# HKUST-KnowComp/DualMessagePassing

Measured on AMD Instinct MI355X. Metric: (pattern,graph) pairs/sec DMPNN fwd+bwd hid=128, higher is better.
Workload: dtype f32

## Files before the change

dualmessagepassing_amd/_abi.py:

```python
import ctypes

c_int = ctypes.c_int
c_i32 = ctypes.c_int32
c_i64 = ctypes.c_int64
c_u64 = ctypes.c_uint64
c_f32 = ctypes.c_float
c_double = ctypes.c_double
c_ptr = ctypes.c_void_p
c_size = ctypes.c_size_t

ABI_VERSION = 97

DMP_COLLATE_MAX_JOBS = 4
DMP_POOL_MAX_JOBS = 4
DMP_REDUCE_MAX_SEGMENTS = 16
DMP_ADAMW_MAX_SKIP = 16
DMP_ADAMW_MAX_SEGMENTS = 1024
DMP_LOOKUP_MAX_JOBS = 8
DMP_CONCAT_MAX_JOBS = 12
DMP_GEMM_MAX_JOBS = 12
DMP_GEMM_MAX_TERMS = 3
DMP_ATB_MAX_JOBS = 8
DMP_MEM_MEAN, DMP_MEM_SUM, DMP_MEM_MAX = 0, 1, 2
DMP_LRP_MAX_NEIGHBOURS = 32
# ... 282 lines not shown
    "dmp_typed_partial_rows": (c_i64, [c_i64, c_int]),
    "dmp_out_fwd_typed": (c_int, [_p(dmp_typed_job), c_int, c_ptr, c_ptr, c_ptr, c_i64, c_i64, c_int, c_ptr]),
    "dmp_bwd_h1_typed": (c_int, [c_ptr, c_i64, c_ptr, c_i64, c_ptr, c_i64, c_ptr, c_ptr, c_ptr, c_i64, c_i64, c_int, c_f32, c_ptr, c_i64,
                                 c_ptr, c_ptr, c_ptr]),
    "dmp_kept_rows_jobs": (c_int, [_p(dmp_kept_job), c_int, c_ptr, c_ptr, c_ptr, c_ptr, c_i64, c_ptr, c_ptr, c_ptr, c_ptr]),
    "dmp_row_mask_bits_jobs": (c_int, [_p(dmp_rowmask_job), c_int, c_ptr]),
    "dmp_atb2_blocks": (c_i64, [c_i64, c_int]),
    "dmp_atb2_jobs": (c_int, [_p(dmp_atb2_job), c_int, c_ptr, c_ptr, c_ptr, c_i64, c_i64, c_int, c_ptr]),
    "dmp_bwd_z_w": (c_int, [c_ptr, c_i64, c_ptr, c_i64, c_ptr, c_i64, c_ptr, c_i64, c_i64, c_ptr, c_i64, c_ptr, c_ptr, c_f32, c_f32,
                            c_ptr, c_ptr, c_ptr, c_i64, c_i64, c_int, c_ptr, c_i64, c_ptr, c_i64, c_ptr, c_ptr]),
    "dmp_out_fwd_typed_codes": (c_int, [_p(dmp_typed_job), c_ptr, c_i64, c_int, c_ptr, c_i64, c_i64, c_i64, c_ptr, c_ptr, c_ptr, c_i64, c_i64, c_int, c_ptr]),
    "dmp_bwd_h1_w_blocks": (c_i64, [c_i64]),
    "dmp_bwd_h1_w": (c_int, [c_ptr, c_i64, c_ptr, c_i64, c_ptr, c_i64, c_ptr, c_ptr, c_i64, c_i64, c_int, c_f32, c_ptr, c_i64,
                             c_ptr, c_ptr, c_ptr, c_ptr]),
    "dmp_node_chain_blocks": (c_i64, [c_i64]),
    "dmp_node_chain_panel_words": (c_i64, []),
    "dmp_node_chain_pack": (c_int, [_p(dmp_chain_panel), c_int, c_ptr, c_ptr]),
    "dmp_node_chain_fwd": (c_int, [c_ptr, c_i64, c_ptr, c_i64, c_ptr, c_ptr, c_ptr, c_int, c_f32, c_ptr, c_ptr, c_i64, c_i64, c_int,
                                   c_ptr, c_i64, c_ptr, c_i64, c_ptr, c_i64, c_ptr]),
    "dmp_node_chain_bwd": (c_int, [c_ptr, c_i64, c_ptr, c_i64, c_ptr, c_i64, c_ptr, c_int, c_f32, c_ptr, c_ptr, c_i64, c_i64, c_int,
                                   c_ptr, c_i64, c_ptr, c_i64, c_ptr, c_i64, c_ptr, c_ptr, c_ptr]),
    "dmp_edge_mlp_fwd": (c_int, [c_ptr, c_i64, c_ptr, c_i64, c_ptr, c_i64, c_i64, c_ptr, c_ptr, c_ptr, c_ptr, c_i64, c_int, c_ptr, c_ptr, c_i64,
                                 c_ptr, c_ptr, c_ptr, c_i64, c_i64, c_int, c_f32, c_ptr, c_i64, c_ptr, c_i64, c_ptr]),
    "dmp_row_mask_bits": (c_int, [c_ptr, c_i64, c_ptr, c_ptr]),
    "dmp_row_mask_rows": (c_int, [c_ptr, c_i64, c_int, c_i64, c_ptr, c_ptr]),
    "dmp_bwd_z_fused": (c_int, [c_ptr, c_i64, c_ptr, c_i64, c_ptr, c_i64, c_i64, c_ptr, c_i64, c_ptr, c_ptr, c_ptr,
                                c_f32, c_f32, c_i64, c_int, c_ptr, c_i64, c_ptr]),
    "dmp_gemm_k128": (c_int, [c_ptr, c_i64, c_ptr, c_i64, c_int, c_ptr, c_i64, c_i64, c_int, c_ptr]),
    "dmp_edge_combine": (c_int, [c_ptr, c_i64, c_ptr, c_i64, c_ptr, c_ptr, c_ptr, c_ptr, c_ptr, c_i64,
                                 c_int, c_int, c_f32, c_ptr, c_i64, c_ptr]),
    "dmp_relu_bwd_g_colsum": (c_int, [c_ptr, c_i64, c_ptr, c_i64, c_ptr, c_ptr, c_i64, c_int, c_f32, c_ptr, c_i64,
                                      c_ptr, c_ptr]),
    "dmp_edge_combine_bwd_g": (c_int, [c_ptr, c_i64, c_ptr, c_ptr, c_i64, c_int, c_ptr, c_i64, c_ptr]),
    "dmp_compgcn_agg": (c_int, [c_ptr, c_i64, c_ptr, c_i64, c_ptr, c_ptr, c_ptr, c_ptr, c_i64, c_int, c_int,
                                c_ptr, c_i64, c_ptr]),
    "dmp_compgcn_agg_bwd": (c_int, [c_ptr, c_i64, c_ptr, c_i64, c_ptr, c_i64, c_ptr, c_ptr, c_ptr, c_ptr,
                                    c_i64, c_int, c_int, c_ptr, c_i64, c_ptr, c_i64, c_ptr]),
    "dmp_attn_supported_dh": (c_int, [c_int]),
    "dmp_attn_fwd": (c_int, [c_ptr, c_ptr, c_ptr, c_ptr, c_ptr, c_i64, c_i64, c_i64, c_int, c_int, c_f32, c_ptr, c_ptr, c_ptr, c_ptr]),
    "dmp_attn_bwd": (c_int, [c_ptr, c_ptr, c_ptr, c_ptr, c_ptr, c_ptr, c_ptr, c_ptr, c_i64, c_i64, c_i64, c_int, c_int, c_f32, c_ptr,
                             c_ptr, c_ptr, c_ptr, c_ptr]),
    "dmp_mem_init_fwd": (c_int, [c_ptr, c_i64, c_ptr, c_i64, c_ptr, c_i64, c_i64, c_int, c_int, c_int, c_int, c_int, c_ptr, c_ptr,
                                 c_ptr, c_ptr, c_ptr, c_ptr, c_ptr]),
    "dmp_mem_init_bwd": (c_int, [c_ptr, c_ptr, c_ptr, c_ptr, c_ptr, c_i64, c_i64, c_int, c_int, c_int, c_int, c_ptr, c_ptr, c_ptr]),
    "dmp_cnn_fwd": (c_int, [c_ptr, c_i64, c_i64, c_int, c_ptr, c_ptr, c_int, c_int, c_int, c_int, c_int, c_f32, c_ptr, c_int, c_ptr,
                            c_ptr, c_ptr, c_ptr, c_ptr]),
# ... 35 lines not shown
```

dualmessagepassing_amd/_build.py:

```python
import fcntl
import hashlib
import os
import shutil
import subprocess
import tempfile

_HERE = os.path.dirname(os.path.abspath(__file__))
CSRC = os.path.join(_HERE, "csrc")
LIB_PATH = os.path.join(CSRC, "libdmp_hip.so")
HASH_PATH = LIB_PATH + ".srchash"
SOURCES = ["dmp_agg.hip", "dmp_segacc.hip", "dmp_compact.hip", "dmp_graph.hip", "dmp_fused.hip", "dmp_mfma.hip", "dmp_typed.hip", "dmp_h1w.hip", "dmp_nodechain.hip", "dmp_edgemlp.hip", "dmp_atb.hip", "dmp_fold.hip", "dmp_heads.hip", "dmp_layer0.hip", "dmp_bn.hip", "dmp_attn.hip", "dmp_mem.hip", "dmp_cnn.hip", "dmp_rnn.hip", "dmp_relconv.hip", "dmp_relcorr.hip", "dmp_txl.hip", "dmp_match.hip", "dmp_lrp.hip", "dmp_rank.hip", "dmp_rank_typed.hip", "dmp_lrppool.hip",
           "dmp_subiso.cpp"]
HEADERS = ["dmp_common.h", "dmp_mfma_common.h", "dmp_rank_kernel.h", os.path.join("..", "..", "include", "dmp_hip.h")]
ARCH = "gfx950"
FLAGS = ["-O3", "-std=c++17", "-fPIC", "-ffp-contract=off", "-Wall", "-Wno-unused-function"]


def find_hipcc():
    for cand in (os.environ.get("HIPCC"), shutil.which("hipcc"), "/opt/rocm/bin/hipcc"):
        if cand and os.path.exists(cand):
            return cand
    return None


def source_hash():
    h = hashlib.sha256()
    h.update((ARCH + " ".join(FLAGS)).encode())
    for f in SOURCES + HEADERS:
        with open(os.path.join(CSRC, f), "rb") as fh:
            h.update(f.encode())
            h.update(fh.read())
    return h.hexdigest()


# ... 53 lines not shown
```

dualmessagepassing_amd/fused.py:

```python
import ctypes as _ctypes
import os as _os
import threading

import torch
from torch.autograd.function import once_differentiable

from . import _abi, _lib, gatememo, ops
from ._lib import check, ptr, stream_ptr


def _partials(rows, H, dev):
    lib = _lib.load()
    return torch.empty((int(lib.dmp_colsum_partial_rows(rows, H)), H), dtype=torch.float32, device=dev)


MAX_REDUCE_SEGMENTS = _abi.DMP_REDUCE_MAX_SEGMENTS


class _Deferred(threading.local):

    def __init__(self):
        self.stack = []


# ... 544 lines not shown

def l0_rows(l0, W0, z):
    if l0 is None or not getattr(l0, "z_from_codes", False):
        return z
    n, K, H = l0.z_head.size(0), l0.K, W0.size(1)
    out = torch.empty((l0.enc.size(0), H), dtype=torch.float32, device=l0.enc.device)
    out[:n].copy_(l0.z_head)
    if out.size(0) > n:
        smallk_embed(l0.enc[n:, :K], W0.detach()[-K:], None, out[n:], H)
    return out


USE_OUT_CODES = True


def out_codes_ok(h1, enc, K, Wc):
    lib = _lib.load()
    lim = (1 << 32) - 65536
    return bool(USE_OUT_CODES and h1.size(1) == 128 and not lib.dmp_dev_get_exact_fp32() and 1 <= K <= 16 and Wc.size(0) == K and Wc.size(1) == 128
                and enc.dtype == torch.float32 and enc.stride(1) == 1 and enc.stride(0) % 4 == 0 and enc.data_ptr() % 16 == 0
                and enc.size(0) == h1.size(0) and h1.size(0) * 128 * 4 < lim and Wc.stride(1) == 1)


def out_fwd_typed_codes(h1, W2t, b2, enc, K, Wc, tiles, prev=None, out=None, w_in_out=True, row0=0):
    lib = _lib.load()
    slot_edge, tile_scale, num_tiles, bound = tiles
    R, H = h1.shape
    if out is None:
        out = dead_rows_buffer((R, H), h1.device)
    Wc = Wc.detach()
    _lib.require_gpu(h1, W2t, out, prev, b2, enc, Wc)
    j = _abi.dmp_typed_job()
    j.Hin, j.ldh, j.W2, j.ldw, j.w_in_out = h1.data_ptr(), h1.stride(0), W2t.data_ptr(), W2t.stride(0), int(bool(w_in_out))
    j.bias = ptr(b2)
    j.R, j.ldr = ptr(prev), (prev.stride(0) if prev is not None else H)
    j.R2, j.ldr2 = None, H
    j.act, j.slope = 0, 0.0
    j.out, j.ldo = out.data_ptr(), out.stride(0)
    with _lib.timed("out_fwd_typed_codes[H=%d,R=%d]", (H, R), 4 * H * R * 2 + 4 * enc.size(1) * R):
        check(lib.dmp_out_fwd_typed_codes(_ctypes.byref(j), ptr(enc), enc.stride(0), int(K), ptr(Wc), Wc.stride(0), int(row0),
                                          0 if prev is None else min(R, prev.size(0)), ptr(slot_edge), ptr(tile_scale),
                                          ptr(num_tiles), bound, R, H, stream_ptr()), "dmp_out_fwd_typed_codes")
    return out


def out_fwd_typed(h1, W2t, b2, prev, tiles, out=None, w_in_out=True, slope=None, prev2=None, first=None):
    R, H = h1.shape
    if out is None:
        out = dead_rows_buffer((R, H), h1.device)
    if first is not None:
        if prev2 is not None or slope is not None:
            raise _lib.DmpError("out_fwd_typed(first=...): neither a second addend nor an activation on the result")
        edge_mlp_fwd(first["z"], first["Wes"], first["P"], first["ldp"], first["bias"], first["coef"], first["index"], first["slope"],
                     W2t, b2, prev, tiles, sel=first.get("sel"), w_in_out=w_in_out, h1=h1, out=out)
        return out
    typed_jobs([dict(a=h1, W=W2t, bias=b2, prev=prev, prev2=prev2, out=out, w_in_out=w_in_out, slope=slope)], tiles)
    return out


USE_EDGE_MLP_FWD = True


def edge_mlp_fwd_ok(H, *tensors):
    if not USE_EDGE_MLP_FWD or H != 128 or _lib.load().dmp_dev_get_exact_fp32():
        return False
    lim = (1 << 32) - 65536
    for a in tensors:
        if a is None:
            continue
        if (a.dtype != torch.float32 or a.dim() != 2 or a.stride(1) != 1 or a.stride(0) % 4 or a.stride(0) * 4 > 16383
                or a.data_ptr() % 16 or a.size(0) * a.stride(0) * 4 >= lim):
            return False
    return True


def edge_mlp_fwd(z, Wes, P, ldp, bias, coef, index, slope, W2t, b2, prev, tiles, sel=None, w_in_out=True, h1=None, out=None):
    lib = _lib.load()
    E, H = z.shape
    slot_edge, tile_scale, num_tiles, bound = tiles
    if h1 is None:
        h1 = dead_rows_buffer((E, H), z.device)
    if out is None:
        out = dead_rows_buffer((E, H), z.device)
    Wes = Wes.contiguous()
    sel_a, sel_b = (sel[0], sel[1]) if sel is not None else index.edge_select(coef)[:2]
    _lib.require_gpu(z, Wes, P, bias, W2t, b2, prev, h1, out)
    with _lib.timed("edge_fwd_typed[H=%d,E=%d]", (H, E), 4 * H * (2 * E + 2 * index.num_nodes) + 12 * E):
        check(lib.dmp_edge_mlp_fwd(ptr(z), z.stride(0), ptr(Wes), Wes.size(1), ptr(P), ldp, index.num_nodes, ptr(bias), ptr(sel_a), ptr(sel_b),
                                   ptr(W2t), W2t.stride(0), int(bool(w_in_out)), ptr(b2), ptr(prev), prev.stride(0) if prev is not None else H,
                                   ptr(slot_edge), ptr(tile_scale), ptr(num_tiles), bound, E, H, float(slope), ptr(h1), h1.stride(0),
                                   ptr(out), out.stride(0), stream_ptr()), "dmp_edge_mlp_fwd")
    return h1, out


def bwd_h1_typed(d_o, W2, h1, tiles, slope=0.0, out=None):
    lib = _lib.load()
# ... 423 lines not shown
    return gatememo.memo(v_gate, "node_rows", (index,), build)


L0_NODE_MAX_COLS = 40


def l0_node_pack(VK, K0, H, Mv, Ma, Mb):
    W = torch.zeros((L0_NODE_MAX_COLS, 3 * H), dtype=torch.float32, device=Mv.device)
    W[:VK] = Mv
    W[VK:VK + K0, :H] = Ma
    W[VK + K0:VK + 2 * K0, :H] = Mb
    return W


def l0_node_fwd(venc, VK, S0, K0, Kp, W, bias, slope, mask, n0, n1, H, h1, P, rows=None, q_begin=0):
    lib = _lib.load()
    lst, cnt = rows if (rows is not None and mask is not None) else (None, None)
    with _lib.timed("l0_node_fwd[K=%d,R=%d]", (VK + 2 * K0, n1 - n0), 4 * (3 * H + VK + 2 * K0) * (n1 - n0)):
        check(lib.dmp_l0_node_fwd(ptr(venc), venc.stride(0), VK, ptr(S0), S0.stride(0), K0, Kp, ptr(W), W.stride(0), ptr(bias), float(slope),
                                  ptr(mask), ptr(lst), ptr(cnt), 0 if lst is None else lst.numel(), min(int(q_begin), n0), n0, n1, H,
                                  ptr(h1), h1.stride(0), ptr(P), P.stride(0), stream_ptr()), "dmp_l0_node_fwd")


def l0_edge_fwd(enc, K, M, P, ldp, bias, coef, index, slope=0.0, rows=None, out=None, mask=None):
    lib = _lib.load()
    E, H = enc.size(0), M.size(1) // 2
    if out is None:
        out = torch.empty((E, H), dtype=torch.float32, device=enc.device)
    r0, r1 = (0, E) if rows is None else rows
    sel_a, sel_b, coef_e = index.edge_select(coef)
    if mask is not None and r0 % 32 != 0:
        mask = None
    if mask is not None and l0_row_list(r0, r1 - r0):
        lst, cnt = kept_rows(mask, r0, r1)
        with _lib.timed("l0_edge_fwd[K=%d,E=%d]", (K, r1 - r0), 4 * H * (r1 - r0 + min(2 * index.num_nodes, 2 * (r1 - r0))) + (4 * enc.size(1) + 12) * (r1 - r0)):
            check(lib.dmp_l0_edge_fwd_rows(ptr(enc[r0:]), enc.stride(0), K, ptr(M), M.stride(0), ptr(P), ldp, ptr(bias), ptr(coef_e[r0:]),
                                           ptr(sel_a[r0:]), ptr(sel_b[r0:]), ptr(lst), ptr(cnt), r1 - r0, H, slope, ptr(out[r0:]),
                                           out.stride(0), stream_ptr()), "dmp_l0_edge_fwd_rows")
        return out
    with _lib.timed("l0_edge_fwd[K=%d,E=%d]", (K, r1 - r0), 4 * H * (r1 - r0 + min(2 * index.num_nodes, 2 * (r1 - r0))) + (4 * enc.size(1) + 12) * (r1 - r0)):
        check(lib.dmp_l0_edge_fwd_masked(ptr(enc[r0:]), enc.stride(0), K, ptr(M), M.stride(0), ptr(P), ldp, ptr(bias), ptr(coef_e[r0:]),
                                         ptr(sel_a[r0:]), ptr(sel_b[r0:]), None if mask is None else ptr(mask[r0 // 32:]), r1 - r0, H,
                                         slope, ptr(out[r0:]), out.stride(0), stream_ptr()),
              "dmp_l0_edge_fwd")
    return out


def l0_bwd_w(enc, K, coef_e, d_pre, d_zn=None, rows=None, out=None, mask=None):
    lib = _lib.load()
    E, H = d_pre.shape
    r0, r1 = (0, E) if rows is None else rows
    own = False
    if mask is not None and r0 % 32 != 0:
# ... 377 lines not shown
        if chained:
            pass
        elif nd is not None:
            xn = dead_rows_buffer((N, H), z.device) if (inner & 1) else torch.zeros((N, H), dtype=torch.float32, device=z.device)
            if nW2t is not None:
                out_fwd_typed(H1n, nW2t, nb2, x if residual else None, nd.tiles, out=xn)
            else:
                out_fwd_typed(H1n, nW2, nb2, x if residual else None, nd.tiles, out=xn, w_in_out=False)
        elif onepanel_ok(H):
            xn = out_fwd_mfma(H1n, nW2, nb2, v_gate, x if residual else None, nW2t)
        else:
            xn = gate_residual(x if residual else None, torch.addmm(nb2, H1n, nW2.t()), v_gate)
        sums_only = epool is not None and not edge_rows
        zn = None
        side.wait("erows" if l0 is not None else "tiles")
        dead_gate = e_gate if dead_h1_rows(index, H, e_gate) else None
        dead_in = dead_gate is not None and dead_edge_rows(index, H, e_gate)
        mlp_tiles = None
        if (l0 is None and dead_in and not sums_only and residual and eW2t is not None and (inner & 1)
                and edge_mlp_fwd_ok(H, z, PXr, eW2t)):
            mlp_tiles = live_tiles(index, coef, e_gate)
        if l0 is not None:
            H1e = dead_rows_buffer((z.size(0), H), z.device) if dead_gate is not None else torch.empty((z.size(0), H), dtype=torch.float32, device=z.device)
            for t, rows, _ in tables:
                if rows[1] > rows[0]:
                    l0_edge_fwd(enc0, K0, M0[t * K0:(t + 1) * K0], PXr, ldpx, be, coef, index, slope, rows, H1e,
                                mask=gate_row_mask(dead_gate) if dead_gate is not None else None)
        elif mlp_tiles is not None:
            H1e = dead_rows_buffer((z.size(0), H), z.device)
            zn = out_fwd_typed(H1e, eW2t, eb2, z, mlp_tiles,
                               first=dict(z=z, Wes=Wes, P=PXr, ldp=ldpx, bias=be, coef=coef, index=index, slope=slope,
                                          sel=None if nd is None else nd.sel))
        elif typed_ok(index, H):
            H1e = edge_fwd_typed(z, Wes, PXr, ldpx, be, coef, index, slope, dead_gate=dead_gate, sel=None if nd is None else nd.sel)
        elif mfma_ok(index, H):
            H1e = edge_fwd_mfma(z, Wes, PXr, ldpx, be, coef, index, slope)
        else:
            G = z @ Wes
            H1e = edge_combine_raw(G, 2 * H, PXr, ldpx, be, coef, index, H, relu=True, slope=slope)
            del G
            if not sums_only:
                Oe = torch.addmm(eb2, H1e, eW2.t())
                zn = gate_residual(z if residual else None, Oe, e_gate)
        if zn is None and not sums_only:
            dead = (3 if (inner & 1) else 1) if dead_in else 0
            side.wait("tiles")
            lt = live_tiles(index, coef, e_gate) if (dead == 3 and eW2t is not None) else None
            if lt is not None:
                tl_ = ascending_tiles(e_gate) or lt
                if l0 is not None and residual and getattr(l0, "z_from_codes", False) and out_codes_ok(H1e, l0.enc, l0.K, W0[-l0.K:]):
# ... 337 lines not shown
```

include/dmp_hip.h:

```cpp
#ifndef DMP_HIP_H
#define DMP_HIP_H

#include <stddef.h>
#include <stdint.h>

#ifdef __cplusplus
extern "C" {
#endif

#define DMP_OK 0
#define DMP_ERR_BAD_ARG (-1)
#define DMP_ERR_UNSUPPORTED (-2)
#define DMP_ERR_HIP (-3)

#define DMP_ABI_VERSION 97
int dmp_abi_version(void);
const char *dmp_last_hip_error(void);


size_t dmp_csr_workspace_words(int64_t num_nodes, int64_t num_edges);

int dmp_csr_build(const int64_t *key, const uint8_t *flag, int64_t num_edges,
                  int64_t num_nodes, int32_t *rowptr, int32_t *ent,
                  int32_t *key32, int64_t *degree, int32_t *status,
// ... 492 lines not shown
                 const int32_t *slot_edge, const int32_t *num_tiles, int64_t tiles_bound, int64_t E, int H, float slope,
                 float *dG, int64_t ldg, float *partial, float *partial_rows, float *partial_w, void *stream);

typedef struct {
  const float *W; int64_t ld; int transposed;
} dmp_chain_panel;
int64_t dmp_node_chain_blocks(int64_t tiles_bound);
int64_t dmp_node_chain_panel_words(void);
int dmp_node_chain_pack(const dmp_chain_panel *panels, int num_panels, uint32_t *out, void *stream);
int dmp_node_chain_fwd(const float *x, int64_t ldx, const float *S, int64_t lds, const uint32_t *panels, const float *bn, const float *b2,
                       int residual, float slope, const int32_t *slot, const int32_t *num_tiles, int64_t tiles_bound, int64_t rows, int H,
                       float *H1n, int64_t ldh, float *P, int64_t ldp, float *xn, int64_t ldxn, void *stream);
int dmp_node_chain_bwd(const float *dxn, int64_t ldd, const float *H1n, int64_t ldh, const float *dP, int64_t ldp, const uint32_t *panels,
                       int residual, float slope, const int32_t *slot, const int32_t *num_tiles, int64_t tiles_bound, int64_t rows, int H,
                       float *dPn, int64_t ldn, float *dS, int64_t lds, float *dx, int64_t ldx, float *partial, float *partial_rows,
                       void *stream);

int dmp_edge_mlp_fwd(const float *Z, int64_t ldz, const float *W, int64_t ldw, const float *P, int64_t ldp, int64_t num_nodes,
                     const float *bias1, const int32_t *selA, const int32_t *selB, const float *W2, int64_t ldw2, int w2_in_out,
                     const float *bias2, const float *R, int64_t ldr, const int32_t *slot_edge, const float *tile_scale,
                     const int32_t *num_tiles, int64_t tiles_bound, int64_t num_edges, int H, float slope, float *H1, int64_t ldh,
                     float *out, int64_t ldo, void *stream);

int dmp_bwd_z_fused(const float *dPre, int64_t ldp, const float *W, int64_t ldw,
                    const float *D, int64_t ldd, int64_t num_nodes, const float *base, int64_t ldb,
                    const float *coefE, const int32_t *dst, const uint8_t *flag, float s0,
                    float s1, int64_t num_edges, int H, float *dZ, int64_t ldz, void *stream);

int dmp_edge_fwd_typed(const float *Z, int64_t ldz, const float *W, int64_t ldw, const float *P,
                       int64_t ldp, int64_t num_nodes, const float *bias, const int32_t *selA,
                       const int32_t *selB, const int32_t *slot_edge, const float *tile_scale,
                       const int32_t *num_tiles, int64_t tiles_bound, int64_t num_edges, int H,
                       float slope, float *H1, int64_t ldh, void *stream);
int dmp_mask_slots(const int32_t *slot, int64_t n, const float *gate, int64_t E, int32_t *out, void *stream);
int dmp_bwd_z_typed_arow(const float *dPre, int64_t ldp, const float *W, int64_t ldw, const float *D, int64_t ldd,
                         int64_t num_nodes, const float *base, int64_t ldb, const int32_t *dst, const uint8_t *flag,
                         float s0, float s1, const int32_t *slot_edge, const int32_t *slot_arow, const float *tile_scale,
                         const int32_t *num_tiles, int64_t tiles_bound, int64_t E, int H, int w_transposed,
                         const int32_t *base_map, int64_t base_rows, float *dZ, int64_t ldz, void *stream);

int64_t dmp_atb_typed_blocks_h(int64_t tiles_bound, int H);
int dmp_atb_typed(const float *Z, int64_t ldz, const float *dPre, int64_t ldp,
                  const int32_t *slot_edge, const float *tile_scale, const int32_t *num_tiles,
                  int64_t tiles_bound, int64_t num_edges, int H, float *partial_T,
                  float *partial_B, void *stream);

// ... 122 lines not shown
```

Before: 487,900.

## Fuse layer-0 edge MLP first and second GEMMs into one warp-specialized kernel

Adds a new HIP kernel that computes the layer-0 edge first linear layer (from code encodings via small per-table matrices plus gathered node projections), activation, and the second linear layer with code term and residual in a single launch. Producer waves build the hidden tile in LDS while consumer waves run the output GEMM on it, using split-bf16 MFMA emulation of fp32. This is meant to remove the separate l0_edge_fwd and out_fwd_typed_codes launches and the intermediate H1 round trip before the second GEMM. The fused path is gated on operand layout, K limits, tile availability and the residual/codes configuration, so some calls fall back to the old path.

```diff
diff --git a/dualmessagepassing_amd/_abi.py b/dualmessagepassing_amd/_abi.py
--- a/dualmessagepassing_amd/_abi.py
+++ b/dualmessagepassing_amd/_abi.py
@@ -328,6 +328,10 @@
                                    c_ptr, c_i64, c_ptr, c_i64, c_ptr, c_i64, c_ptr, c_ptr, c_ptr]),
     "dmp_edge_mlp_fwd": (c_int, [c_ptr, c_i64, c_ptr, c_i64, c_ptr, c_i64, c_i64, c_ptr, c_ptr, c_ptr, c_ptr, c_i64, c_int, c_ptr, c_ptr, c_i64,
                                  c_ptr, c_ptr, c_ptr, c_i64, c_i64, c_int, c_f32, c_ptr, c_i64, c_ptr, c_i64, c_ptr]),
+    "dmp_l0_edge_mlp_max_codes": (c_int, []),
+    "dmp_l0_edge_mlp_fwd": (c_int, [c_ptr, c_i64, c_int, c_ptr, c_i64, c_int, c_i64, c_ptr, c_i64, c_i64, c_ptr, c_ptr, c_ptr, c_ptr, c_f32,
+                                    c_ptr, c_i64, c_int, c_ptr, c_ptr, c_i64, c_i64, c_ptr, c_i64, c_i64, c_ptr, c_ptr, c_i64, c_i64, c_int,
+                                    c_ptr, c_i64, c_ptr, c_i64, c_ptr]),
     "dmp_row_mask_bits": (c_int, [c_ptr, c_i64, c_ptr, c_ptr]),
     "dmp_row_mask_rows": (c_int, [c_ptr, c_i64, c_int, c_i64, c_ptr, c_ptr]),
     "dmp_bwd_z_fused": (c_int, [c_ptr, c_i64, c_ptr, c_i64, c_ptr, c_i64, c_i64, c_ptr, c_i64, c_ptr, c_ptr, c_ptr,
diff --git a/dualmessagepassing_amd/_build.py b/dualmessagepassing_amd/_build.py
--- a/dualmessagepassing_amd/_build.py
+++ b/dualmessagepassing_amd/_build.py
@@ -9,7 +9,7 @@
 CSRC = os.path.join(_HERE, "csrc")
 LIB_PATH = os.path.join(CSRC, "libdmp_hip.so")
 HASH_PATH = LIB_PATH + ".srchash"
-SOURCES = ["dmp_agg.hip", "dmp_segacc.hip", "dmp_compact.hip", "dmp_graph.hip", "dmp_fused.hip", "dmp_mfma.hip", "dmp_typed.hip", "dmp_h1w.hip", "dmp_nodechain.hip", "dmp_edgemlp.hip", "dmp_atb.hip", "dmp_fold.hip", "dmp_heads.hip", "dmp_layer0.hip", "dmp_bn.hip", "dmp_attn.hip", "dmp_mem.hip", "dmp_cnn.hip", "dmp_rnn.hip", "dmp_relconv.hip", "dmp_relcorr.hip", "dmp_txl.hip", "dmp_match.hip", "dmp_lrp.hip", "dmp_rank.hip", "dmp_rank_typed.hip", "dmp_lrppool.hip",
+SOURCES = ["dmp_agg.hip", "dmp_segacc.hip", "dmp_compact.hip", "dmp_graph.hip", "dmp_fused.hip", "dmp_mfma.hip", "dmp_typed.hip", "dmp_h1w.hip", "dmp_nodechain.hip", "dmp_edgemlp.hip", "dmp_l0mlp.hip", "dmp_atb.hip", "dmp_fold.hip", "dmp_heads.hip", "dmp_layer0.hip", "dmp_bn.hip", "dmp_attn.hip", "dmp_mem.hip", "dmp_cnn.hip", "dmp_rnn.hip", "dmp_relconv.hip", "dmp_relcorr.hip", "dmp_txl.hip", "dmp_match.hip", "dmp_lrp.hip", "dmp_rank.hip", "dmp_rank_typed.hip", "dmp_lrppool.hip",
            "dmp_subiso.cpp"]
 HEADERS = ["dmp_common.h", "dmp_mfma_common.h", "dmp_rank_kernel.h", os.path.join("..", "..", "include", "dmp_hip.h")]
 ARCH = "gfx950"
diff --git a/dualmessagepassing_amd/csrc/dmp_l0mlp.hip b/dualmessagepassing_amd/csrc/dmp_l0mlp.hip
--- /dev/null
+++ b/dualmessagepassing_amd/csrc/dmp_l0mlp.hip
@@ -0,0 +1,378 @@
+#include <type_traits>
+
+#include "dmp_mfma_common.h"
+
+namespace dmp {
+namespace {
+
+struct L0MlpArgs {
+  const float *enc; int64_t lde; int K;
+  const float *M; int64_t ldm; int tables;
+  int64_t row_split;
+  const float *P; int64_t ldp; int64_t num_nodes;
+  const float *bias1;
+  const float *coef_e;
+  const int32_t *selA, *selB;
+  const float *W2; int64_t ldw2; int w2_transposed;
+  const float *bias2;
+  const float *Wc; int64_t ldwc; int64_t code_row0;
+  const float *R; int64_t ldr; int64_t r_rows;
+  float *H1; int64_t ldh;
+  float *out; int64_t ldo;
+  int64_t E;
+  const int32_t *slot_edge;
+  const int32_t *num_tiles;
+  float slope;
+};
+
+constexpr int kHL = 128, kThreadsL = 512;
+constexpr int kStrideL = (kHL + 8) / 2;
+constexpr int kPlaneL = kSub * kStrideL;
+constexpr int kTileL = 3 * kPlaneL;
+constexpr int kSlot = 12;
+constexpr int kOpGroups = 4 * kSlot / 16;
+constexpr int kOpStride = (4 * kSlot + 8) / 2;
+constexpr int kOpPlane = kSub * kOpStride;
+constexpr int kOpTile = 3 * kOpPlane;
+constexpr int kCxPlane = kSub * 8;
+constexpr int kCxTile = 3 * kCxPlane;
+constexpr int kRingL = 4;
+constexpr int kOpOff = 2 * kTileL * 4;
+constexpr int kCxOff = kOpOff + 2 * kOpTile * 4;
+constexpr int kScrOffL = kCxOff + kRingL * kCxTile * 4;
+constexpr int kRowsOffL = kScrOffL + 8 * 32 * kScrStride * 4;
+constexpr int kL0MlpLdsBytes = kRowsOffL + 3 * kRingL * kSub * 4;
+constexpr int kHalfL = kHL / 2, kGroupsL = kHalfL / 8;
+static_assert(4 * kSlot % 16 == 0 && kOpStride % 4 == 0, "whole k-groups, 16-byte fragment reads");
+
+__global__ __launch_bounds__(kThreadsL, 1) void l0_edge_mlp_k(const L0MlpArgs p) {
+  extern __shared__ __attribute__((aligned(16))) unsigned char lds[];
+  uint32_t *const himg = reinterpret_cast<uint32_t *>(lds);
+  uint32_t *const opimg = reinterpret_cast<uint32_t *>(lds + kOpOff);
+  uint32_t *const cximg = reinterpret_cast<uint32_t *>(lds + kCxOff);
+  uint32_t *const rowA = reinterpret_cast<uint32_t *>(lds + kRowsOffL);
+  uint32_t *const rowB = rowA + kRingL * kSub, *const rowC = rowB + kRingL * kSub;
+  const int wave = __builtin_amdgcn_readfirstlane((int)(threadIdx.x >> 6));
+  const bool second = wave >= 4;
+  const int lane = threadIdx.x & 63, li = lane & 31, h = lane >> 5, cs = wave & 3;
+  const int gtid = threadIdx.x & 255;
+  const int col = 32 * cs + li;
+  float *const scr = reinterpret_cast<float *>(lds + kScrOffL) + wave * (32 * kScrStride);
+  const int lrow = lane >> 3, c4 = 32 * cs + (lane & 7) * 4;
+  const uint32_t col4 = (uint32_t)c4 * 4u;
+  constexpr uint32_t kRowBytes = kHL * 4u;
+  constexpr uint32_t kNone = 0xFFFFFFFFu, kOOB = 0xFFFFF000u;
+
+  const int ntiles = __builtin_amdgcn_readfirstlane(*p.num_tiles);
+  const int chunk = (ntiles + (int)gridDim.x - 1) / (int)gridDim.x;
+  const int lo = (int)blockIdx.x * chunk;
+  const int hi = lo + chunk < ntiles ? lo + chunk : ntiles;
+  const int mine = hi > lo ? hi - lo : 0;
+  if (mine == 0) return;
+
+  Split8 B6[kGroupsL];
+  f32x16 acc;
+  auto six = [&](const Frag8 &ah, const Frag8 &am, const Frag8 &al, const Split8 &bb) {
+    acc = __builtin_amdgcn_mfma_f32_32x32x16_bf16(al.v, bb.hi.v, acc, 0, 0, 0);
+    acc = __builtin_amdgcn_mfma_f32_32x32x16_bf16(ah.v, bb.lo.v, acc, 0, 0, 0);
+    acc = __builtin_amdgcn_mfma_f32_32x32x16_bf16(am.v, bb.mid.v, acc, 0, 0, 0);
+    acc = __builtin_amdgcn_mfma_f32_32x32x16_bf16(am.v, bb.hi.v, acc, 0, 0, 0);
+    acc = __builtin_amdgcn_mfma_f32_32x32x16_bf16(ah.v, bb.mid.v, acc, 0, 0, 0);
+    acc = __builtin_amdgcn_mfma_f32_32x32x16_bf16(ah.v, bb.hi.v, acc, 0, 0, 0);
+  };
+  auto x6_tile = [&](const uint32_t *ar, int plane, int step, auto groups) {
+    constexpr int G = decltype(groups)::value;
+#pragma unroll
+    for (int r = 0; r < 16; ++r) acc[r] = 0.f;
+    Frag8 ah, am, al;
+    ah.v = *reinterpret_cast<const bf16x8 *>(ar);
+    am.v = *reinterpret_cast<const bf16x8 *>(ar + plane);
+    al.v = *reinterpret_cast<const bf16x8 *>(ar + 2 * plane);
+#pragma unroll
+    for (int g = 0; g < G; ++g) {
+      Frag8 nh = ah, nm = am, nl = al;
+      if (g + 1 < G) {
+        nh.v = *reinterpret_cast<const bf16x8 *>(ar + step * (g + 1));
+        nm.v = *reinterpret_cast<const bf16x8 *>(ar + plane + step * (g + 1));
+        nl.v = *reinterpret_cast<const bf16x8 *>(ar + 2 * plane + step * (g + 1));
+      }
+      __builtin_amdgcn_sched_barrier(0);
+      six(ah, am, al, B6[g]);
+      __builtin_amdgcn_sched_barrier(0);
+      ah = nh; am = nm; al = nl;
+    }
+  };
+  auto acc_to_scr = [&]() {
+#pragma unroll
+    for (int r = 0; r < 16; ++r) scr[((r & 3) + 8 * (r >> 2) + 4 * h) * kScrStride + li] = acc[r];
+  };
+
+  if (!second) {
+    const float4 bias4 = buf_load4(make_rsrc(p.bias1, p.bias1 ? kRowBytes : 0u), col4, 0);
+    const float slope = __builtin_bit_cast(float, __builtin_amdgcn_readfirstlane(__builtin_bit_cast(int, p.slope)));
+    const uint32_t rows4 = (uint32_t)(p.E * 4);
+    const srsrc_t rs_enc = make_srsrc(p.enc, p.lde, p.E);
+    const srsrc_t rs_H1 = make_srsrc(p.H1, p.ldh, p.E);
+    const srsrc_t rs_T = make_srsrc(p.P, p.ldp, p.num_nodes);
+    const rsrc_t rs_idxA = make_rsrc(p.selA, rows4);
+    const rsrc_t rs_idxB = make_rsrc(p.selB, rows4);
+    const rsrc_t rs_coef = make_rsrc(p.coef_e, rows4);
+    const rsrc_t rs_slot = make_rsrc(p.slot_edge, (uint32_t)ntiles * (kSub * 4u));
+    const int cq = gtid & 3, crow = (gtid >> 2) & (kSub - 1);
+    const bool stager = gtid < 4 * kSub, owner = gtid < kSub;
+    const bool cload = stager && 4 * cq < kSlot && 4 * cq < (int)p.lde;
+    const uint32_t slot_c = stager ? (uint32_t)crow * 4u : kOOB, slot_o = owner ? (uint32_t)gtid * 4u : kOOB;
+    const int K = __builtin_amdgcn_readfirstlane(p.K);
+
+    auto load_panel = [&]() {
+      const rsrc_t rs_M = make_rsrc(p.M, (uint32_t)((int64_t)p.tables * K * p.ldm * 4));
+      float w[kOpGroups][8];
+#pragma unroll
+      for (int g = 0; g < kOpGroups; ++g) {
+#pragma unroll
+        for (int j = 0; j < 8; ++j) {
+          const int k = 16 * g + 8 * h + j, s = k / kSlot, jj = k - s * kSlot, t = s & 1, half = s >> 1;
+          const bool ok = jj < K && t < p.tables;
+          const uint32_t off = ok ? (uint32_t)(((int64_t)(t * K + jj) * p.ldm + half * kHL + col) * 4) : kOOB;
+          w[g][j] = __uint_as_float(__builtin_amdgcn_raw_buffer_load_b32(rs_M, (int)off, 0, 0));
+        }
+      }
+#pragma unroll
+      for (int g = 0; g < kOpGroups; ++g)
+        split8(make_float4(w[g][0], w[g][1], w[g][2], w[g][3]), make_float4(w[g][4], w[g][5], w[g][6], w[g][7]), B6[g]);
+    };
+
+    int id_c = -1, id_own = -1;
+    int id_data = -1, own_staged = -1;
+    float4 pre_c = make_float4(0.f, 0.f, 0.f, 0.f);
+    float pre_cf = 0.f;
+    uint32_t pre_a = 0, pre_b = 0;
+    int raw_c = -1, raw_own = -1;
+    bool ids_ok = false;
+    auto load_ids = [&](int k) {
+      ids_ok = k < mine;
+      const uint32_t so = (uint32_t)(lo + (ids_ok ? k : mine - 1)) * (kSub * 4u);
+      raw_c = (int)__builtin_amdgcn_raw_buffer_load_b32(rs_slot, (int)slot_c, (int)so, 0);
+      raw_own = (int)__builtin_amdgcn_raw_buffer_load_b32(rs_slot, (int)slot_o, (int)so, 0);
+    };
+    auto load_data = [&]() {
+      id_c = (ids_ok && stager) ? raw_c : -1;
+      id_own = (ids_ok && owner) ? raw_own : -1;
+      pre_c = sbuf_load4(rs_enc, cload ? id_c : -1, (uint32_t)cq * 16u);
+      pre_cf = __uint_as_float(__builtin_amdgcn_raw_buffer_load_b32(rs_coef, (int)(id_c >= 0 ? (uint32_t)id_c * 4u : kOOB), 0, 0));
+      const uint32_t eo = id_own >= 0 ? (uint32_t)id_own * 4u : kOOB;
+      pre_a = __builtin_amdgcn_raw_buffer_load_b32(rs_idxA, (int)eo, 0, 0);
+      pre_b = __builtin_amdgcn_raw_buffer_load_b32(rs_idxB, (int)eo, 0, 0);
+      id_data = id_c;
+      own_staged = id_own;
+    };
+    auto stage = [&](int buf, int par) {
+      if (stager) {
+        const int kc = K - 4 * cq;
+        const float x0 = kc > 0 ? pre_c.x : 0.f, x1 = kc > 1 ? pre_c.y : 0.f, x2 = kc > 2 ? pre_c.z : 0.f, x3 = kc > 3 ? pre_c.w : 0.f;
+        uint2 xh, xm, xl, yh, ym, yl;
+        split_pair(x0, x1, xh.x, xm.x, xl.x);
+        split_pair(x2, x3, xh.y, xm.y, xl.y);
+        split_pair(pre_cf * x0, pre_cf * x1, yh.x, ym.x, yl.x);
+        split_pair(pre_cf * x2, pre_cf * x3, yh.y, ym.y, yl.y);
+        const uint2 zero = make_uint2(0u, 0u);
+        const bool t1 = (int64_t)id_data >= p.row_split;
+        if (4 * cq < kSlot) {
+          uint32_t *q = opimg + buf * kOpTile + crow * kOpStride + 2 * cq;
+#pragma unroll
+          for (int s = 0; s < 4; ++s) {
+            const bool mineslot = ((s & 1) != 0) == t1;
+            const uint2 vh = (s >> 1) ? yh : xh, vm = (s >> 1) ? ym : xm, vl = (s >> 1) ? yl : xl;
+            *reinterpret_cast<uint2 *>(q + (kSlot / 2) * s) = mineslot ? vh : zero;
+            *reinterpret_cast<uint2 *>(q + (kSlot / 2) * s + kOpPlane) = mineslot ? vm : zero;
+            *reinterpret_cast<uint2 *>(q + (kSlot / 2) * s + 2 * kOpPlane) = mineslot ? vl : zero;
+          }
+        }
+        const bool cz = (int64_t)id_data >= p.code_row0;
+        uint32_t *c = cximg + par * kCxTile + crow * 8 + 2 * cq;
+        *reinterpret_cast<uint2 *>(c) = cz ? xh : zero;
+        *reinterpret_cast<uint2 *>(c + kCxPlane) = cz ? xm : zero;
+        *reinterpret_cast<uint2 *>(c + 2 * kCxPlane) = cz ? xl : zero;
+      }
+      if (owner) {
+        const bool ok = own_staged >= 0;
+        rowA[par * kSub + gtid] = ok ? pre_a : kNone;
+        rowB[par * kSub + gtid] = ok ? pre_b : kNone;
+        rowC[par * kSub + gtid] = ok ? (uint32_t)own_staged : kNone;
+      }
+    };
+    float4 g0[4], g1[4];
+    auto fetch_operand = [&](int par, int k) {
+      const int rr = 8 * k + lrow;
+      g0[k] = sbuf_load4(rs_T, (int)rowA[par * kSub + rr], col4);
+      g1[k] = sbuf_load4(rs_T, (int)rowB[par * kSub + rr], col4 + kRowBytes);
+    };
+    auto epilogue = [&](int k, int par) {
+      uint32_t *const img = himg + (k & 1) * kTileL;
+      const int nxt = (par + 1) & (kRingL - 1);
+      acc_to_scr();
+#pragma unroll
+      for (int q = 0; q < 4; ++q) {
+        const int rr = 8 * q + lrow;
+        float4 v = *reinterpret_cast<const float4 *>(&scr[rr * kScrStride + (lane & 7) * 4]);
+        v.x = act_fwd((v.x + (g0[q].x - g1[q].x)) + bias4.x, slope);
+        v.y = act_fwd((v.y + (g0[q].y - g1[q].y)) + bias4.y, slope);
+        v.z = act_fwd((v.z + (g0[q].z - g1[q].z)) + bias4.z, slope);
+        v.w = act_fwd((v.w + (g0[q].w - g1[q].w)) + bias4.w, slope);
+        const uint32_t rc = rowC[par * kSub + rr];
+        sbuf_store4(v, rs_H1, (int)rc, col4);
+        const bool pad = rc == kNone;
+        uint2 ph, pm, pl;
+        split_pair(pad ? 0.f : v.x, pad ? 0.f : v.y, ph.x, pm.x, pl.x);
+        split_pair(pad ? 0.f : v.z, pad ? 0.f : v.w, ph.y, pm.y, pl.y);
+        uint32_t *w = img + rr * kStrideL + (c4 >> 1);
+        *reinterpret_cast<uint2 *>(w) = ph;
+        *reinterpret_cast<uint2 *>(w + kPlaneL) = pm;
+        *reinterpret_cast<uint2 *>(w + 2 * kPlaneL) = pl;
+        fetch_operand(nxt, q);
+      }
+    };
+
+    load_ids(0);
+    load_data();
+    load_ids(1);
+    load_panel();
+    stage(0, 0);
+    load_data();
+    load_ids(2);
+    lds_barrier();
+#pragma unroll
+    for (int c = 0; c < 4; ++c) fetch_operand(0, c);
+    for (int k = 0; k < mine; ++k) {
+      const int par = k & (kRingL - 1);
+      stage((k + 1) & 1, (par + 1) & (kRingL - 1));
+      load_data();
+      load_ids(k + 3);
+      x6_tile(opimg + (k & 1) * kOpTile + li * kOpStride + 4 * h, kOpPlane, 8, std::integral_constant<int, kOpGroups>());
+      lds_barrier();
+      epilogue(k, par);
+    }
+    lds_barrier();
+  } else {
+    __builtin_amdgcn_s_setprio(1);
+    const float4 bias4 = buf_load4(make_rsrc(p.bias2, p.bias2 ? kRowBytes : 0u), col4, 0);
+    const srsrc_t rs_R = make_srsrc(p.R, p.R ? p.ldr : (int64_t)kHL, p.r_rows);
+    const srsrc_t rs_O = make_srsrc(p.out, p.ldo, p.E);
+    Split8 BX;
+    {
+      const rsrc_t rs_Wc = make_rsrc(p.Wc, (uint32_t)((int64_t)p.K * p.ldwc * 4));
+      float w[8];
+#pragma unroll
+      for (int j = 0; j < 8; ++j)
+        w[j] = __uint_as_float(__builtin_amdgcn_raw_buffer_load_b32(rs_Wc, (int)(((int64_t)(8 * h + j) * p.ldwc + col) * 4), 0, 0));
+      const rsrc_t rs_W = make_rsrc(p.W2, (uint32_t)(kHL * p.ldw2 * 4));
+      const uint32_t w_first = (uint32_t)(p.w2_transposed ? (int64_t)col * p.ldw2 + kHalfL * h : (int64_t)kHalfL * h * p.ldw2 + col) * 4u;
+      const uint32_t w_step = __builtin_amdgcn_readfirstlane((int)(p.w2_transposed ? 4 : p.ldw2 * 4));
+      uint32_t off;
+      asm volatile("v_mov_b32 %0, %1" : "=v"(off) : "v"(w_first));
+#pragma unroll
+      for (int s0 = 0; s0 < kHalfL; s0 += 32) {
+        float w0[32];
+#pragma unroll
+        for (int j = 0; j < 32; ++j) w0[j] = __uint_as_float(__builtin_amdgcn_raw_buffer_load_b32(rs_W, (int)off, (int)((s0 + j) * w_step), 0));
+        if (s0 == 0) split8(make_float4(w[0], w[1], w[2], w[3]), make_float4(w[4], w[5], w[6], w[7]), BX);
+#pragma unroll
+        for (int q = 0; q < 32; q += 8)
+          split8(make_float4(w0[q], w0[q + 1], w0[q + 2], w0[q + 3]), make_float4(w0[q + 4], w0[q + 5], w0[q + 6], w0[q + 7]), B6[(s0 + q) / 8]);
+        __builtin_amdgcn_sched_barrier(0);
+      }
+    }
+    float4 g1[4];
+    auto fetch_residual = [&](int par, int q) {
+      g1[q] = sbuf_load4(rs_R, (int)rowC[par * kSub + 8 * q + lrow], col4);
+    };
+    lds_barrier();
+#pragma unroll
+    for (int q = 0; q < 4; ++q) fetch_residual(0, q);
+    lds_barrier();
+    for (int k = 0; k < mine; ++k) {
+      const int par = k & (kRingL - 1), nxt = (par + 1) & (kRingL - 1);
+      lds_barrier();
+      x6_tile(himg + (k & 1) * kTileL + li * kStrideL + (kHalfL / 2) * h, kPlaneL, 4, std::integral_constant<int, kGroupsL>());
+      {
+        const uint32_t *c = cximg + par * kCxTile + li * 8 + 4 * h;
+        Frag8 ch, cm, cl;
+        ch.v = *reinterpret_cast<const bf16x8 *>(c);
+        cm.v = *reinterpret_cast<const bf16x8 *>(c + kCxPlane);
+        cl.v = *reinterpret_cast<const bf16x8 *>(c + 2 * kCxPlane);
+        six(ch, cm, cl, BX);
+      }
+      acc_to_scr();
+#pragma unroll
+      for (int q = 0; q < 4; ++q) {
+        const int rr = 8 * q + lrow;
+        float4 v = *reinterpret_cast<const float4 *>(&scr[rr * kScrStride + (lane & 7) * 4]);
+        v.x = (v.x + bias4.x) + g1[q].x; v.y = (v.y + bias4.y) + g1[q].y;
+        v.z = (v.z + bias4.z) + g1[q].z; v.w = (v.w + bias4.w) + g1[q].w;
+        sbuf_store4(v, rs_O, (int)rowC[par * kSub + rr], col4);
+        fetch_residual(nxt, q);
+      }
+    }
+  }
+}
+
+inline unsigned l0_mlp_blocks(int64_t tiles_bound) {
+  const int64_t cap = 256;
+  return (unsigned)(tiles_bound < cap ? (tiles_bound > 0 ? tiles_bound : 1) : cap);
+}
+
+constexpr int kMaxDevicesL = 64;
+inline bool l0_mlp_lds_ready() {
+  static bool done[kMaxDevicesL] = {};
+  int dev = 0;
+  if (hipGetDevice(&dev) != hipSuccess || dev < 0 || dev >= kMaxDevicesL) dev = 0;
+  if (done[dev]) return true;
+  const hipError_t e = hipFuncSetAttribute(reinterpret_cast<const void *>(&l0_edge_mlp_k), hipFuncAttributeMaxDynamicSharedMemorySize, kL0MlpLdsBytes);
+  if (e != hipSuccess) { set_last_hip_error(e); return false; }
+  done[dev] = true;
+  return true;
+}
+
+}
+}
+
+using namespace dmp;
+
+extern "C" {
+
+int dmp_l0_edge_mlp_max_codes(void) { return kSlot; }
+
+int dmp_l0_edge_mlp_fwd(const float *enc, int64_t lde, int K, const float *M, int64_t ldm, int tables, int64_t row_split, const float *P,
+                        int64_t ldp, int64_t num_nodes, const float *bias1, const float *coef_e, const int32_t *selA, const int32_t *selB,
+                        float slope, const float *W2, int64_t ldw2, int w2_in_out, const float *bias2, const float *Wc, int64_t ldwc,
+                        int64_t code_row0, const float *R, int64_t ldr, int64_t r_rows, const int32_t *slot_edge, const int32_t *num_tiles,
+                        int64_t tiles_bound, int64_t E, int H, float *H1, int64_t ldh, float *out, int64_t ldo, void *stream) {
+  if (H != 128 || g_exact_fp32) return DMP_ERR_UNSUPPORTED;
+  if (E < 0 || num_nodes < 0 || tiles_bound < 0 || K < 1 || tables < 1 || row_split < 0 || code_row0 < 0 || code_row0 > E || r_rows < 0 || r_rows > E)
+    return DMP_ERR_BAD_ARG;
+  if (K > kSlot || tables > 2 || !slope_ok(slope)) return DMP_ERR_UNSUPPORTED;
+  if (E == 0 || tiles_bound == 0) return DMP_OK;
+  if (!enc || !M || !P || !coef_e || !selA || !selB || !W2 || !Wc || !slot_edge || !num_tiles || !H1 || !out || lde < K || ldm < 2 * H ||
+      ldp < 2 * H || ldw2 < H || ldwc < H || ldh < H || ldo < H || (R && ldr < H))
+    return DMP_ERR_BAD_ARG;
+  if (lde % 4 || ldh % 4 || ldp % 4 || ldo % 4 || (R && ldr % 4) || !aligned16(enc) || !aligned16(H1) || !aligned16(P) || !aligned16(out) ||
+      (R && !aligned16(R)) || (bias1 && !aligned16(bias1)) || (bias2 && !aligned16(bias2)))
+    return DMP_ERR_UNSUPPORTED;
+  const int64_t lim32 = ((int64_t)1 << 32) - 8192;
+  if (!stride_ok(lde) || !stride_ok(ldh) || !stride_ok(ldp) || !stride_ok(ldo) || (R && !stride_ok(ldr)) || E >= ((int64_t)1 << 30) ||
+      num_nodes >= ((int64_t)1 << 31) || tiles_bound * kSub * 4 >= lim32 || (int64_t)tables * K * ldm * 4 >= lim32 ||
+      (int64_t)H * ldw2 * 4 >= lim32 || (int64_t)K * ldwc * 4 >= lim32 || !fits4g(E, lde) || !fits4g(E, ldh) || !fits4g(E, ldo) ||
+      (R && !fits4g(r_rows, ldr)) || !fits4g(num_nodes, ldp))
+    return DMP_ERR_UNSUPPORTED;
+  if (!l0_mlp_lds_ready()) return DMP_ERR_HIP;
+  L0MlpArgs a{};
+  a.enc = enc; a.lde = lde; a.K = K; a.M = M; a.ldm = ldm; a.tables = tables; a.row_split = tables == 1 ? E : row_split;
+  a.P = P; a.ldp = ldp; a.num_nodes = num_nodes; a.bias1 = bias1; a.coef_e = coef_e; a.selA = selA; a.selB = selB;
+  a.W2 = W2; a.ldw2 = ldw2; a.w2_transposed = w2_in_out ? 0 : 1; a.bias2 = bias2; a.Wc = Wc; a.ldwc = ldwc; a.code_row0 = code_row0;
+  a.R = R; a.ldr = R ? ldr : H; a.r_rows = R ? r_rows : 0; a.H1 = H1; a.ldh = ldh; a.out = out; a.ldo = ldo; a.E = E;
+  a.slot_edge = slot_edge; a.num_tiles = num_tiles; a.slope = slope;
+  l0_edge_mlp_k<<<l0_mlp_blocks(tiles_bound), kThreadsL, kL0MlpLdsBytes, (hipStream_t)stream>>>(a);
+  return check_launch();
+}
+
+}
diff --git a/dualmessagepassing_amd/fused.py b/dualmessagepassing_amd/fused.py
--- a/dualmessagepassing_amd/fused.py
+++ b/dualmessagepassing_amd/fused.py
@@ -590,13 +590,18 @@
                 and enc.size(0) == h1.size(0) and h1.size(0) * 128 * 4 < lim and Wc.stride(1) == 1)
 
 
-def out_fwd_typed_codes(h1, W2t, b2, enc, K, Wc, tiles, prev=None, out=None, w_in_out=True, row0=0):
+def out_fwd_typed_codes(h1, W2t, b2, enc, K, Wc, tiles, prev=None, out=None, w_in_out=True, row0=0, first=None):
     lib = _lib.load()
     slot_edge, tile_scale, num_tiles, bound = tiles
     R, H = h1.shape
     if out is None:
         out = dead_rows_buffer((R, H), h1.device)
     Wc = Wc.detach()
+    if first is not None:
+        l0_edge_fwd(enc, K, first["M"], first["P"], first["ldp"], first["bias"], first["coef"], first["index"], first["slope"], out=h1,
+                    mlp=dict(tables=first["tables"], split=first["split"], W2t=W2t, b2=b2, Wc=Wc, row0=row0, prev=prev, tiles=tiles,
+                             w_in_out=w_in_out, out=out))
+        return out
     _lib.require_gpu(h1, W2t, out, prev, b2, enc, Wc)
     j = _abi.dmp_typed_job()
     j.Hin, j.ldh, j.W2, j.ldw, j.w_in_out = h1.data_ptr(), h1.stride(0), W2t.data_ptr(), W2t.stride(0), int(bool(w_in_out))
@@ -630,7 +635,11 @@
 
 
 def edge_mlp_fwd_ok(H, *tensors):
-    if not USE_EDGE_MLP_FWD or H != 128 or _lib.load().dmp_dev_get_exact_fp32():
+    return bool(USE_EDGE_MLP_FWD and _one_launch_mlp_operands_ok(H, tensors))
+
+
+def _one_launch_mlp_operands_ok(H, tensors):
+    if H != 128 or _lib.load().dmp_dev_get_exact_fp32():
         return False
     lim = (1 << 32) - 65536
     for a in tensors:
@@ -640,6 +649,14 @@
                 or a.data_ptr() % 16 or a.size(0) * a.stride(0) * 4 >= lim):
             return False
     return True
+
+
+USE_L0_EDGE_MLP = True
+
+
+def l0_edge_mlp_ok(H, K, tables, *tensors):
+    return bool(USE_L0_EDGE_MLP and 1 <= tables <= 2 and 1 <= K <= _lib.load().dmp_l0_edge_mlp_max_codes()
+                and _one_launch_mlp_operands_ok(H, tensors))
 
 
 def edge_mlp_fwd(z, Wes, P, ldp, bias, coef, index, slope, W2t, b2, prev, tiles, sel=None, w_in_out=True, h1=None, out=None):
@@ -1109,13 +1126,27 @@
                                   ptr(h1), h1.stride(0), ptr(P), P.stride(0), stream_ptr()), "dmp_l0_node_fwd")
 
 
-def l0_edge_fwd(enc, K, M, P, ldp, bias, coef, index, slope=0.0, rows=None, out=None, mask=None):
+def l0_edge_fwd(enc, K, M, P, ldp, bias, coef, index, slope=0.0, rows=None, out=None, mask=None, mlp=None):
     lib = _lib.load()
     E, H = enc.size(0), M.size(1) // 2
     if out is None:
         out = torch.empty((E, H), dtype=torch.float32, device=enc.device)
     r0, r1 = (0, E) if rows is None else rows
     sel_a, sel_b, coef_e = index.edge_select(coef)
+    if mlp is not None:
+        slot_edge, _, num_tiles, bound = mlp["tiles"]
+        W2t, b2, Wc, prev, zn = mlp["W2t"], mlp["b2"], mlp["Wc"], mlp["prev"], mlp["out"]
+        tables = int(mlp["tables"])
+        split = int(mlp["split"]) if tables == 2 else 0
+        _lib.require_gpu(enc, M, P, bias, W2t, b2, Wc, prev, out, zn)
+        with _lib.timed("l0_edge_fwd[K=%d,E=%d]", (K, E - split), 4 * H * (E + min(2 * index.num_nodes, 2 * E)) + (4 * enc.size(1) + 12) * E):
+            check(lib.dmp_l0_edge_mlp_fwd(ptr(enc), enc.stride(0), int(K), ptr(M), M.stride(0), tables, split, ptr(P), ldp, index.num_nodes,
+                                          ptr(bias), ptr(coef_e), ptr(sel_a), ptr(sel_b), float(slope), ptr(W2t), W2t.stride(0),
+                                          int(bool(mlp.get("w_in_out", True))), ptr(b2), ptr(Wc), Wc.stride(0), int(mlp["row0"]), ptr(prev),
+                                          prev.stride(0) if prev is not None else H, 0 if prev is None else min(E, prev.size(0)),
+                                          ptr(slot_edge), ptr(num_tiles), bound, E, H, ptr(out), out.stride(0), ptr(zn), zn.stride(0),
+                                          stream_ptr()), "dmp_l0_edge_mlp_fwd")
+        return out
     if mask is not None and r0 % 32 != 0:
         mask = None
     if mask is not None and l0_row_list(r0, r1 - r0):
@@ -1539,10 +1570,26 @@
             mlp_tiles = live_tiles(index, coef, e_gate)
         if l0 is not None:
             H1e = dead_rows_buffer((z.size(0), H), z.device) if dead_gate is not None else torch.empty((z.size(0), H), dtype=torch.float32, device=z.device)
-            for t, rows, _ in tables:
-                if rows[1] > rows[0]:
-                    l0_edge_fwd(enc0, K0, M0[t * K0:(t + 1) * K0], PXr, ldpx, be, coef, index, slope, rows, H1e,
-                                mask=gate_row_mask(dead_gate) if dead_gate is not None else None)
+            l0_tiles = None
+            if (not sums_only and residual and eW2t is not None and getattr(l0, "z_from_codes", False)
+                    and out_codes_ok(H1e, l0.enc, l0.K, W0[-l0.K:])
+                    and l0_edge_mlp_ok(H, K0, W0.size(0) // K0, enc0, PXr, eW2t, l0.z_head)):
+                if dead_in and (inner & 1):
+                    side.wait("tiles")
+                    lt = live_tiles(index, coef, e_gate)
+                    if lt is not None:
+                        l0_tiles = ascending_tiles(e_gate) or lt
+                elif e_gate is None:
+                    l0_tiles = identity_tiles(H1e.size(0), H1e.device)
+            if l0_tiles is not None:
+                zn = out_fwd_typed_codes(H1e, eW2t, eb2, l0.enc, l0.K, W0[-l0.K:], l0_tiles, prev=l0.z_head, row0=l0.z_head.size(0),
+                                         first=dict(M=M0, tables=W0.size(0) // K0, split=l0.esplit, P=PXr, ldp=ldpx, bias=be, coef=coef,
+                                                    index=index, slope=slope))
+            else:
+                for t, rows, _ in tables:
+                    if rows[1] > rows[0]:
+                        l0_edge_fwd(enc0, K0, M0[t * K0:(t + 1) * K0], PXr, ldpx, be, coef, index, slope, rows, H1e,
+                                    mask=gate_row_mask(dead_gate) if dead_gate is not None else None)
         elif mlp_tiles is not None:
             H1e = dead_rows_buffer((z.size(0), H), z.device)
             zn = out_fwd_typed(H1e, eW2t, eb2, z, mlp_tiles,
diff --git a/include/dmp_hip.h b/include/dmp_hip.h
--- a/include/dmp_hip.h
+++ b/include/dmp_hip.h
@@ -538,6 +538,13 @@
                      const int32_t *num_tiles, int64_t tiles_bound, int64_t num_edges, int H, float slope, float *H1, int64_t ldh,
                      float *out, int64_t ldo, void *stream);
 
+int dmp_l0_edge_mlp_max_codes(void);
+int dmp_l0_edge_mlp_fwd(const float *enc, int64_t lde, int K, const float *M, int64_t ldm, int tables, int64_t row_split, const float *P,
+                        int64_t ldp, int64_t num_nodes, const float *bias1, const float *coefE, const int32_t *selA, const int32_t *selB,
+                        float slope, const float *W2, int64_t ldw2, int w2_in_out, const float *bias2, const float *Wc, int64_t ldwc,
+                        int64_t code_row0, const float *R, int64_t ldr, int64_t r_rows, const int32_t *slot_edge, const int32_t *num_tiles,
+                        int64_t tiles_bound, int64_t num_edges, int H, float *H1, int64_t ldh, float *out, int64_t ldo, void *stream);
+
 int dmp_bwd_z_fused(const float *dPre, int64_t ldp, const float *W, int64_t ldw,
                     const float *D, int64_t ldd, int64_t num_nodes, const float *base, int64_t ldb,
                     const float *coefE, const int32_t *dst, const uint8_t *flag, float s0,
```

After: 495,100 (median of 6 runs). 1.01x the previous value.
